# JosephCatrambone/aruco3

Hardware: AMD Instinct MI355X
Metric: frames/sec at 1920x1080 ARUCO dict (higher is better)
Workload: dtype u8

## Files before the change

aruco3_amd/_lib.py:

```python
import ctypes as C
from pathlib import Path

import numpy as np

import os

_HERE = Path(__file__).resolve().parent
LIB_PATH = Path(os.environ["A3_HIP_LIB"]).resolve() if os.environ.get("A3_HIP_LIB") else _HERE / "libaruco3_hip.so"

OK, ERR_INVALID, ERR_HIP, ERR_CAPACITY, ERR_INTERNAL, ERR_NO_DEVICE, ERR_LIMIT = 0, -1, -2, -3, -4, -5, -6
FMT_RGB8, FMT_RGBA8, FMT_L8, FMT_BGRA8 = 0, 1, 2, 3
MEM_HOST, MEM_DEVICE = 0, 1
PROFILE_OFF, PROFILE_STAGES, PROFILE_THRESHOLD_ONLY, PROFILE_THRESHOLD_SAMPLED = 0, 1, 2, 3
STAGE_THRESHOLD, STAGE_CONTOUR, STAGE_DECODE = 0, 1, 2
STEP_WHOLE, STEP_DECODE_DEFERRED, STEP_HELD_RELEASED_BY_LAST, STEP_HELD_RELEASED_EARLY, STEP_BURST_LAST, STEP_HELD = 0, 1, 2, 3, 4, 5
REFINE_NONE, REFINE_SUBPIX = 0, 1
BOARD_NONE, BOARD_OK = 0, 1
BOARD_MAX_MARKERS = 1024
DIST_NONE, DIST_RATIONAL = 0, 1
CHARUCO_MAX_CORNERS = 2048
CHARUCO_NO_ADJ = 0xFFFFFFFF
CALIB_FIX_PRINCIPAL_POINT, CALIB_ZERO_TANGENT_DIST, CALIB_FIX_K3, CALIB_RATIONAL_MODEL, CALIB_USE_INTRINSIC_GUESS = 1, 2, 4, 8, 16
CALIB_OK, CALIB_TOO_FEW, CALIB_NO_INIT, CALIB_NOT_FINITE = 1, 2, 3, 4
CALIB_VIEW_USED, CALIB_VIEW_TOO_FEW_POINTS, CALIB_VIEW_DEGENERATE = 1, 2, 3
# ... 6 lines not shown
STEP_NAMES = {0: "whole", 1: "decode_deferred", 2: "held_released_by_last", 3: "held_released_early", 4: "burst_last", 5: "held"}

SYMBOLS = [
    "a3_abi_version", "a3_default_config", "a3_create", "a3_destroy", "a3_last_error", "a3_set_stream", "a3_get_stream", "a3_set_pool_limits",
    "a3_get_tau", "a3_order_after", "a3_set_debug_taps", "a3_detect_batch", "a3_detect_batch_pose", "a3_detect_batch_submit", "a3_detect_batch_collect", "a3_detect_batch_pose_submit", "a3_detect_batch_pose_collect",
    "a3_host_alloc", "a3_host_free", "a3_host_register", "a3_host_unregister", "a3_get_stats", "a3_synth_render", "a3_download_grey", "a3_download_thresholded",
    "a3_candidate_count", "a3_download_candidates", "a3_download_homographies", "a3_estimate_pose", "a3_estimate_pose_normalized",
    "a3_find_nearest", "a3_calculate_tau", "a3_set_profiling", "a3_get_profile",
    "a3_contour_count", "a3_download_contours", "a3_detection_record_bytes", "a3_pack_detections",
    "a3_default_refine_config", "a3_set_corner_refinement", "a3_get_refined_corners", "a3_refine_corners",
    "a3_set_board", "a3_get_board_poses", "a3_estimate_board_pose",
    "a3_default_distortion", "a3_set_distortion", "a3_get_undistorted_corners", "a3_undistort_points",
    "a3_default_charuco_config", "a3_set_charuco", "a3_get_charuco_corners", "a3_get_charuco_poses", "a3_interpolate_charuco",
    "a3_calibrate_cameras", "a3_calibrate_rigs",
]
INTERNAL_SYMBOLS = ["a3_debug_set_overlap", "a3_debug_build_flags", "a3_debug_spin", "a3_debug_set_hold", "a3_debug_set_jump_rounds", "a3_debug_launch_threshold", "a3_debug_kernel_time", "a3_selftest_ieee", "a3_debug_clockwise", "a3_debug_rotate_bits", "a3_debug_discard_too_near", "a3_debug_inject_candidates"]


class A3Error(RuntimeError):
    def __init__(self, code, message):
        super().__init__(f"aruco3_hip error {code}: {message}")
        self.code = code


class Config(C.Structure):
    _fields_ = [
        ("threshold_window", C.c_uint32),
        ("contour_simplification_epsilon", C.c_double),
        ("min_side_length_factor", C.c_float),
        ("min_corner_separation_factor", C.c_float),
        ("homography_sample_size", C.c_uint32),
# ... 180 lines not shown
    L.a3_synth_render.restype = C.c_int
    L.a3_synth_render.argtypes = [C.c_int, vp, vp, C.c_uint32, vp, C.c_uint32, C.c_uint32, C.c_uint32, C.c_int, C.c_float, C.c_float, C.c_int,
                                  vp, C.c_size_t, C.c_size_t]
    if hasattr(L, "a3_debug_set_overlap"):
        L.a3_debug_set_overlap.restype = C.c_int
        L.a3_debug_set_overlap.argtypes = [C.c_int]
    if hasattr(L, "a3_debug_launch_threshold"):
        L.a3_debug_launch_threshold.restype = C.c_int
        L.a3_debug_launch_threshold.argtypes = [vp, vp, C.c_int, C.c_uint32, C.c_uint32, C.c_uint32]
    if hasattr(L, "a3_debug_set_hold"):
        L.a3_debug_set_hold.restype = C.c_int
        L.a3_debug_set_hold.argtypes = [C.c_int]
    if hasattr(L, "a3_debug_set_jump_rounds"):
        L.a3_debug_set_jump_rounds.restype = C.c_int
        L.a3_debug_set_jump_rounds.argtypes = [C.c_int]
    if hasattr(L, "a3_debug_spin"):
        L.a3_debug_spin.restype = C.c_int
        L.a3_debug_spin.argtypes = [vp, C.c_int, C.c_int, C.c_int]
    if hasattr(L, "a3_debug_build_flags"):
        L.a3_debug_build_flags.restype = C.c_int
        L.a3_debug_build_flags.argtypes = []
    L.a3_debug_kernel_time.restype = C.c_int
    L.a3_debug_kernel_time.argtypes = [vp, C.c_int, C.c_int, C.c_int, C.POINTER(C.c_float)]
    L.a3_get_stats.restype = C.c_int
    L.a3_get_stats.argtypes = [vp, C.POINTER(Stats)]
    L.a3_download_grey.restype = C.c_int
    L.a3_download_grey.argtypes = [vp, C.c_uint32, u8p]
    L.a3_download_thresholded.restype = C.c_int
    L.a3_download_thresholded.argtypes = [vp, C.c_uint32, u8p]
    L.a3_candidate_count.restype = C.c_int
# ... 546 lines not shown
```

aruco3_amd/csrc/a3_api.hip:

```cpp
#include <algorithm>
#include <atomic>
#include <cmath>
#include <chrono>
#include <cstddef>
#include <cstdio>
#include <cstring>
#include <mutex>
#include <string>
#include <vector>

#include "a3_common.h"
#include "a3_internal.h"

namespace a3 {
hipError_t launch_grey_threshold(hipStream_t, const uint8_t*, int, size_t, size_t, int, int, uint32_t, uint32_t, uint8_t*, uint64_t*, uint16_t*);
bool threshold_writes_grey_plane(uint32_t radius, const uint8_t* pixels, size_t row_stride, size_t frame_stride, int W);
hipError_t launch_dart_count(hipStream_t, const uint64_t*, int, int, uint32_t, uint32_t, unsigned long long*, uint32_t*, uint64_t, uint32_t*, uint32_t*, void*, size_t);
size_t tile_darts_bytes(uint32_t W, uint32_t H, uint32_t n_frames);
size_t tile_off_offset(uint32_t W, uint32_t H, uint32_t n_frames);
size_t tile_mask_offset_bytes(uint32_t W, uint32_t H, uint32_t n_frames);
hipError_t launch_dart_build(hipStream_t, const uint64_t*, int, int, uint32_t, uint32_t, const uint32_t*, const uint32_t*, uint32_t*, const uint32_t*,
                             uint64_t*, uint32_t*, uint32_t, const uint32_t*, int, const unsigned long long*);
hipError_t launch_zero(hipStream_t, void*, size_t);
size_t entry_state_bytes();
bool finalize_inline(bool frame_entries, bool trust_natural);
size_t fin_state_bytes();
size_t entry_slots(uint32_t);
size_t leader_list_bytes(uint32_t);
hipError_t launch_rank_cycles(hipStream_t, uint32_t, int, const uint64_t*, const uint32_t*,
                              uint32_t*, unsigned int*, void*, void*, void*, uint32_t*, unsigned int*, int, DeviceCounters*, const uint32_t*, int,
                              const uint32_t*, uint32_t*, uint32_t, int, uint32_t, unsigned int*, int);
hipError_t launch_resolve(hipStream_t, const void*, uint32_t, int, const uint64_t*, const uint32_t*, const unsigned int*, uint64_t*, uint64_t*,
                          DeviceCounters*, int, const uint32_t*);
hipError_t launch_select_scatter(hipStream_t, const void*, uint32_t, const uint32_t*, const unsigned int*, const uint32_t*, const uint64_t*,
                                 const uint32_t*, uint32_t, uint32_t,
                                 uint32_t, double, double, ContourRec*, uint32_t*, uint32_t, uint64_t, DeviceCounters*,
                                 const uint64_t*, uint32_t*, const uint32_t*, int, uint32_t*, int, const void*);
// ... 123 lines not shown
    int back_rc = 0;
    bool allow_defer = false;
    int batch_mode = 0;
    std::atomic<uint32_t> stepping{0};
    uint32_t released_others = 0;
    uint32_t reruns = 0;
    a3_config cfg{};
    uint8_t num_bits = 0, tau = 0;
    uint32_t n_codes = 0, mark_size = 0;
    std::string err;

    uint64_t max_darts = kMaxDartsDefault, max_points = kMaxPointsDefault;
    uint32_t max_contours = kMaxContoursDefault;
    uint32_t max_cand = kMaxCandDefault;
    int jump_rounds_hint = 10, resolve_iters_hint = 4;
    uint32_t dbg_nd = 0, dbg_frames = 0, dbg_chunks = 0;
    PixelSrc dbg_src{};
    std::vector<CandRec> inject;
    bool inject_armed = false;
    uint32_t inject_count = 0;
    Batch batch;
    bool pending_trivial = false;
    int resolve_full_ttl = 0;
    int entry_global_ttl = 0;
    bool plan_valid = false, force_host_plan = false;
    uint32_t plan_n = 0, plan_W = 0, plan_H = 0;
    uint64_t plan_darts = 0;
    bool debug_taps = false;
    uint32_t patch_cap = 0;
    bool grey_valid = false;
// ... 131 lines not shown
    A3_HIP(ctx->t_next.ensure(darts * 8));
    A3_HIP(ctx->leader_list.ensure(leader_list_bytes((uint32_t)darts)));
    A3_HIP(ctx->leader_keep.ensure(leader_list_bytes((uint32_t)darts)));
    const size_t eslots = entry_slots((uint32_t)darts);
    A3_HIP(ctx->entry_list.ensure(eslots * 4));
    A3_HIP(ctx->es_a.ensure(eslots * entry_state_bytes()));
    A3_HIP(ctx->es_b.ensure(eslots * entry_state_bytes()));
    return A3_OK;
}

struct DeviceStreams { hipStream_t decode = nullptr, copy = nullptr; };
std::mutex g_streams_mu;
DeviceStreams g_dev_streams[64];
bool g_hold_rests = true;
std::atomic<int> g_jump_rounds_cap{0};
enum { kStreamCopy = 0, kStreamDecode = 1 };

hipError_t create_stream(hipStream_t* st) { return hipStreamCreateWithPriority(st, hipStreamNonBlocking, 0); }

hipError_t device_stream(int device, int kind, hipStream_t* out) {
    std::lock_guard<std::mutex> lk(g_streams_mu);
    DeviceStreams& ds = g_dev_streams[device & 63];
    hipStream_t& st = kind == kStreamDecode ? ds.decode : ds.copy;
    if (!st) {
        const hipError_t e = create_stream(&st);
        if (e != hipSuccess) { st = nullptr; return e; }
    }
    *out = st;
    return hipSuccess;
}
// ... 347 lines not shown
    };
    std::vector<Chunk> chunks;
    std::vector<uint64_t> fd;
    if (device_plan) {
        if (int rc = ensure_chain_buffers(ctx, st, b, cap_d)) return rc;
        chunks.push_back(Chunk{0, n, cap_d, (uint32_t)std::min<uint64_t>(cap_d, 0xFFFFFFFFu)});
        A3_HIP(layout_zero_block(1, n, false));
        ctx->frame_darts_ptr = ctx->frame_darts_dev.as<unsigned long long>();
    } else {
        A3_HIP(ctx->tile_darts.ensure(tile_darts_bytes(W, H, n)));
        ctx->frame_darts_ptr = ctx->frame_darts.as<unsigned long long>();
        A3_HIP(hipMemsetAsync(ctx->frame_darts.p, 0, (size_t)n * 8, st));
    }
    A3_HIP(launch_dart_count(st, ctx->bin.as<uint64_t>(), (int)W, (int)H, 0, n, ctx->frame_darts_ptr, ctx->tile_darts.as<uint32_t>(), cap_d,
                             device_plan ? ctx->frame_base.as<uint32_t>() : nullptr, device_plan ? ctx->scratch_u32 + 8 : nullptr,
                             device_plan ? zero_p : nullptr, device_plan ? zero_bytes : 0));
    const uint32_t* n_live = device_plan ? ctx->scratch_u32 + 8 : nullptr;
    uint32_t max_chunk_frames = n;
    if (!device_plan) {
        if (int rc = ensure_pinned(ctx, std::max<size_t>((size_t)n * 8, 1 << 16))) return rc;
        A3_HIP(hipMemcpyAsync(ctx->pinned, ctx->frame_darts.p, (size_t)n * 8, hipMemcpyDeviceToHost, st));
        A3_HIP(wait_stream(st));
        fd.assign((uint64_t*)ctx->pinned, (uint64_t*)ctx->pinned + n);
        uint64_t biggest = 0;
        for (uint64_t v : fd) { biggest = std::max(biggest, v); ctx->stats.darts += v; }
        if (biggest > kHardMaxDarts) return fail(ctx, A3_ERR_LIMIT, "a frame needs more contour-graph nodes than 32-bit indices allow");
        if (biggest > ctx->max_darts) ctx->max_darts = biggest;
        Chunk c{0, 0, 0, 0};
        for (uint32_t f = 0; f < n; f++) {
            if (c.count && (c.darts + fd[f] > ctx->max_darts || c.count >= kMaxChunkFrames)) { chunks.push_back(c); c = Chunk{f, 0, 0, 0}; }
            c.count++; c.darts += fd[f]; c.max_frame_darts = (uint32_t)std::max<uint64_t>(c.max_frame_darts, fd[f]);
// ... 34 lines not shown
    const int resolve_iters = ctx->resolve_full_ttl > 0 ? ctx->resolve_iters_hint : 0;
    const int inline_resolve_W = ctx->resolve_full_ttl > 0 ? 0 : (int)W;
    const int keep_all = b.taps ? 1 : 0;
    int rounds_max = 0;
    for (size_t ci = 0; ci < chunks.size(); ci++) {
        const Chunk& c = chunks[ci];
        DeviceCounters* ctr = ctx->counters + ci;
        const uint32_t* fb = ctx->frame_base.as<uint32_t>() + ci * (max_chunk_frames + 1);
        const uint32_t nd = (uint32_t)c.darts;
        if (nd == 0) continue;
        if (ci > 0) {
            A3_HIP(hipMemsetAsync(d_leader_count, 0, 4 * 32, st));
            A3_HIP(hipMemsetAsync(ctx->frame_cursor, 0, (size_t)c.count * 4, st));
        }
        const uint32_t* tile_off = ctx->tile_darts.as<uint32_t>() + tile_off_offset(W, H, n);
        A3_HIP(launch_dart_build(st, d_bin, (int)W, (int)H, c.first, c.count, fb, tile_off, ctx->pix_base.as<uint32_t>(),
                                 ctx->tile_darts.as<uint32_t>(), ctx->d_xy.as<uint64_t>(), ctx->d_succ.as<uint32_t>(), nd, n_live, 0,
                                 reinterpret_cast<const unsigned long long*>(ctx->tile_darts.as<uint8_t>() + tile_mask_offset_bytes(W, H, n))));
        int rounds = 1;
        while ((1ull << rounds) < (uint64_t)c.max_frame_darts && rounds < 31) rounds++;
        rounds += 1;
        rounds = std::min(rounds, ctx->jump_rounds_hint);
        if (const int cap = g_jump_rounds_cap.load(std::memory_order_relaxed); cap > 0 && ctx->jump_rounds_hint < 32) rounds = std::min(rounds, cap);
        rounds_max = std::max(rounds_max, rounds);
        uint32_t* const frame_entries = ctx->entry_global_ttl > 0 ? nullptr : ctx->frame_cursor;
        const bool dense_graph = (uint64_t)nd * 10u >= (uint64_t)c.count * npx;
        unsigned int* const dead_ctr = (keep_all || !dense_graph) ? nullptr : d_dead_count;
        A3_HIP(launch_rank_cycles(st, nd, (int)W, ctx->d_xy.as<uint64_t>(), ctx->d_succ.as<uint32_t>(),
                                  ctx->entry_list.as<uint32_t>(), d_entry_count, ctx->es_a.p, ctx->es_b.p,
                                  ctx->fin.p, ctx->leader_list.as<uint32_t>(), d_leader_count, rounds, ctr, n_live, 0, fb,
                                  frame_entries, c.count, 1, min_edge_length, dead_ctr, inline_resolve_W > 0 ? 1 : 0));
        if (rel_mode == 2) { if (int rc = release_waiting()) return rc; }
        ctx->dbg_nd = nd; ctx->dbg_frames = c.count; ctx->dbg_chunks = (uint32_t)chunks.size();
// ... 63 lines not shown
    const float* h_undist = reinterpret_cast<const float*>(hp + head_bytes + (size_t)guess * (sizeof(a3_marker) + pose_bytes + refine_bytes) + board_bytes);
    const float* h_undist_res = h_undist + (size_t)guess * 8;
    {
        std::lock_guard<std::mutex> lk(g_defer_mu);
        if (int rc = flush_deferred_locked(ctx, nullptr)) return rc;
        if (const int rc = ctx->back_rc) { ctx->back_rc = 0; return rc; }
    }
    A3_HIP(wait_event(ctx->ev[4], st));
    const unsigned int* hs = reinterpret_cast<const unsigned int*>(hp);
    const DeviceCounters* hc = reinterpret_cast<const DeviceCounters*>(hp + 256);
    if (b.device_plan) {
        if (hs[9]) { ctx->force_host_plan = true; return 1; }
        ctx->stats.darts = hs[8];
        ctx->dbg_nd = hs[8];
        ctx->plan_darts = hs[8];
    } else {
        ctx->plan_valid = n_chunks == 1;
        ctx->plan_n = n; ctx->plan_W = b.W; ctx->plan_H = b.H;
        ctx->plan_darts = n_chunks == 1 ? b.chunk0_darts : 0;
    }
    unsigned int flags = hs[4];
    for (int sh = 0; sh < 16; sh++) ctx->stats.contours_traced += hs[48 + sh];
    uint64_t need_points = 0; uint32_t need_contours = 0;
    bool jump_short = false, resolve_needed = false, entry_overflow = false;
    for (size_t ci = 0; ci < n_chunks; ci++) {
        flags |= hc[ci].err_flags;
        resolve_needed |= hc[ci].resolve_needed != 0;
        entry_overflow |= hc[ci].entry_overflow != 0;
        need_points = std::max<uint64_t>(need_points, hc[ci].points);
        need_contours = std::max(need_contours, hc[ci].contours);
        ctx->stats.contours_traced += hc[ci].traced;
// ... 582 lines not shown
    struct EventPair {
        hipEvent_t e0 = nullptr, e1 = nullptr;
        ~EventPair() { if (e0) (void)hipEventDestroy(e0); if (e1) (void)hipEventDestroy(e1); }
    } evp;
    A3_HIP(hipEventCreate(&evp.e0)); A3_HIP(hipEventCreate(&evp.e1));
    const hipEvent_t e0 = evp.e0, e1 = evp.e1;
    double total = 0.0;
    unsigned int* d_entry_count = ctx->scratch_u32 + 32;
    unsigned int* d_leader_count = ctx->scratch_u32 + 16;
    for (int r = 0; r < reps; r++) {
        A3_HIP(hipMemsetAsync(d_leader_count, 0, 4 * 32, st));
        A3_HIP(hipEventRecord(e0, st));
        if (kernel == 0) {
            A3_HIP(hipMemsetAsync(ctx->frame_darts.p, 0, (size_t)ctx->frames * 8, st));
            A3_HIP(launch_dart_count(st, ctx->bin.as<uint64_t>(), (int)ctx->W, (int)ctx->H, 0, ctx->frames, ctx->frame_darts.as<unsigned long long>(),
                                     ctx->tile_darts.as<uint32_t>(), 0, nullptr, nullptr, nullptr, 0));
        } else if (kernel == 1) {
            A3_HIP(launch_dart_build(st, ctx->bin.as<uint64_t>(), (int)ctx->W, (int)ctx->H, 0, ctx->dbg_frames, ctx->frame_base.as<uint32_t>(),
                                     ctx->tile_darts.as<uint32_t>() + tile_off_offset(ctx->W, ctx->H, ctx->frames), ctx->pix_base.as<uint32_t>(),
                                     ctx->tile_darts.as<uint32_t>(), ctx->d_xy.as<uint64_t>(),
                                     ctx->d_succ.as<uint32_t>(), ctx->dbg_nd, nullptr, dbg ? dbg : 5,
                                     reinterpret_cast<const unsigned long long*>(ctx->tile_darts.as<uint8_t>() + tile_mask_offset_bytes(ctx->W, ctx->H, ctx->frames))));
        } else if (kernel == 2) {
            A3_HIP(launch_rank_cycles(st, ctx->dbg_nd, (int)ctx->W, ctx->d_xy.as<uint64_t>(), ctx->d_succ.as<uint32_t>(),
                                      ctx->entry_list.as<uint32_t>(),
                                      d_entry_count, ctx->es_a.p, ctx->es_b.p, ctx->fin.p,
                                      ctx->leader_list.as<uint32_t>(), d_leader_count, 0, ctx->counters, nullptr, dbg ? dbg : 11, ctx->frame_base.as<uint32_t>(), nullptr, ctx->dbg_frames, 0,
                                      0u, nullptr, 0));
        } else if (kernel == 3 || kernel == 4) {
            if (kernel == 4) {
                const size_t sweep = std::min<size_t>(ctx->pix_base.cap & ~(size_t)15, (size_t)512 << 20);
                if (sweep) A3_HIP(launch_zero(st, ctx->pix_base.p, sweep));
                A3_HIP(hipEventRecord(e0, st));
            }
            A3_HIP(launch_decode(st, ctx->dbg_src, (int)ctx->W, (int)ctx->H, 0, ctx->fin_xy.as<uint16_t>(), ctx->work.as<uint32_t>(), ctx->scratch_u32,
                                 ctx->max_cand, ctx->cfg.homography_sample_size, ctx->mark_size, ctx->cfg.homography_sample_size, ctx->dict.as<uint64_t>(),
                                 ctx->n_codes, ctx->tau, ctx->cfg.filter_high_bit_errors, ctx->proj.p, ctx->wtab.as<float>(), ctx->outs.p, nullptr, 0u, nullptr, 4096,
// ... 46 lines not shown
    return A3_OK;
}

int a3_debug_set_hold(int on) {
    std::lock_guard<std::mutex> lk(g_defer_mu);
    if (!g_held.empty()) return A3_ERR_INVALID;
    g_hold_rests = on != 0;
    return A3_OK;
}

int a3_debug_set_jump_rounds(int rounds) {
    if (rounds < 0 || rounds > 32) return A3_ERR_INVALID;
    g_jump_rounds_cap.store(rounds, std::memory_order_relaxed);
    return A3_OK;
}

int a3_synth_render(int device, void* hip_stream, const a3_synth_frame* frames, uint32_t n_frames, const a3_synth_marker* markers,
                    uint32_t n_markers, uint32_t width, uint32_t height, int paper, float black, float white, int supersample,
                    void* out_rgb_device, size_t row_stride, size_t frame_stride) {
    if (!frames || !out_rgb_device || (n_markers && !markers) || supersample < 1 || supersample > 8) return A3_ERR_INVALID;
    if (n_frames == 0 || width == 0 || height == 0) return A3_OK;
    if (row_stride == 0) row_stride = (size_t)width * 3;
    if (frame_stride == 0) frame_stride = row_stride * height;
    if (row_stride < (size_t)width * 3 || frame_stride < row_stride * (height - 1) + (size_t)width * 3 || height > 65535 || n_frames > 65535)
        return A3_ERR_INVALID;
    for (uint32_t f = 0; f < n_frames; f++)
        if ((uint64_t)frames[f].first_marker + frames[f].n_markers > n_markers) return A3_ERR_INVALID;
    for (uint32_t m = 0; m < n_markers; m++)
        if (markers[m].n == 0 || markers[m].n > 11) return A3_ERR_INVALID;
    if (hipSetDevice(device) != hipSuccess) return A3_ERR_NO_DEVICE;
// ... 859 lines not shown
```

aruco3_amd/csrc/a3_internal.h:

```cpp
#ifndef ARUCO3_HIP_INTERNAL_H
#define ARUCO3_HIP_INTERNAL_H

#include "../../include/aruco3_hip.h"

#ifdef __cplusplus
extern "C" {
#endif

int  a3_debug_kernel_time(a3_ctx *ctx, int kernel, int dbg, int reps, float *avg_ms);

int  a3_debug_set_overlap(int mode);

int  a3_debug_spin(void *hip_stream, int workgroups, int threads, int usec);

int  a3_debug_set_hold(int on);

int  a3_debug_set_jump_rounds(int rounds);

int  a3_debug_launch_threshold(a3_ctx *ctx, const void *pixels_device, int fmt, uint32_t width, uint32_t height, uint32_t n_frames);

int  a3_debug_build_flags(void);

int  a3_selftest_ieee(a3_ctx *ctx, const double *a, const double *b, size_t n, double *sqrt_a, double *a_div_b,
                      float *sqrtf_a, float *a_divf_b);

int  a3_debug_clockwise(a3_ctx *ctx, const int32_t *quads_xy, size_t n, int32_t *out_xy);
int  a3_debug_rotate_bits(a3_ctx *ctx, const uint8_t *bits, uint32_t n, uint32_t times, uint8_t *out);
int  a3_debug_inject_candidates(a3_ctx *ctx, const uint32_t *quads_xy, size_t n);
int  a3_debug_discard_too_near(a3_ctx *ctx, const uint32_t *quads_xy, size_t n, float min_distance, uint32_t *out_xy, size_t *n_out);

#ifdef __cplusplus
}
#endif
// ... 2 lines not shown
```

aruco3_amd/csrc/k_contours.hip:

```cpp
#include <algorithm>

#include "a3_common.h"


namespace a3 {

constexpr int kFinB = 8;
constexpr int kScatB = 1;

struct Nb8 { uint64_t c; uint64_t n[8]; };

__device__ __forceinline__ uint64_t ldw(const uint64_t* __restrict__ img, int wpr, int H, int j, int y) {
    return (y >= 0 && y < H && j >= 0 && j < wpr) ? img[(size_t)y * wpr + j] : 0ull;
}

__device__ __forceinline__ void pdart_words(const Nb8& nb, uint64_t p[8]) {
#pragma unroll
    for (int k = 0; k < 8; k++) {
        uint64_t m = nb.c & nb.n[k] & ~nb.n[(k + 7) & 7];
        if ((k & 1) == 0) m &= ~nb.n[(k + 6) & 7];
        p[k] = m;
    }
}

// ... 56 lines not shown
    r.n[1] = (a << 1) | (al >> 63);
    r.n[2] = a;
    r.n[3] = (a >> 1) | (ar << 63);
    r.n[4] = (c >> 1) | (cr << 63);
    r.n[5] = (b >> 1) | (br << 63);
    r.n[6] = b;
    r.n[7] = (b << 1) | (bl >> 63);
    return r;
}

constexpr int kCountLanes = 60;
constexpr int kCountHalves = 4;
template <int G>
__global__ __launch_bounds__(64) void k_dart_count(const uint64_t* __restrict__ bits, int W, int H, uint32_t first_frame,
                                                   unsigned long long* __restrict__ frame_darts, uint32_t* __restrict__ tile_darts,
                                                   uint32_t* __restrict__ tile_darts_h1, unsigned long long* __restrict__ tile_mask) {
    static_assert(kCountLanes % kTileWords == 0, "a wave counts whole tiles");
    static_assert((kTileRows / kCountHalves) * kTileWords == 64, "one 64-bit mask per tile and part");
    constexpr int kGroups = 64 / G, kOwners = G == 64 ? kCountLanes : 30, kTilesPerGroup = (kOwners + kTileWords - 1) / kTileWords;
    __shared__ uint32_t s_tile[kGroups][kTilesPerGroup];
    __shared__ unsigned long long s_mask[kGroups][kTilesPerGroup];
    constexpr uint32_t kQ = 128;
    __shared__ uint64_t q_c[kQ], q_up[kQ], q_dn[kQ];
    __shared__ uint32_t q_meta[kQ];
    const int wpr = (int)words_per_row((uint32_t)W);
    const uint32_t f = blockIdx.y;
    const uint32_t tiles_x = dart_tiles_x((uint32_t)W), tiles_y = ((uint32_t)H + kTileRows - 1) / kTileRows;
    const int chunks_x = G == 64 ? (wpr + kCountLanes - 1) / kCountLanes : 1;
    const int lane = threadIdx.x, gl = lane & (G - 1), grp = lane / G;
    const int cx = blockIdx.x % chunks_x, ty = (blockIdx.x / chunks_x) * kGroups + grp;
    const int j = cx * kOwners + gl - 1;
    const bool owner = gl >= 1 && gl <= kOwners && j < wpr && ty < (int)tiles_y;
    const uint64_t* img = bits + (size_t)(first_frame + f) * wpr * H;
    if (lane < kGroups * kTilesPerGroup) { (&s_tile[0][0])[lane] = 0; (&s_mask[0][0])[lane] = 0ull; }
    constexpr int kRows = kTileRows / kCountHalves;
    const int y0 = ty * kTileRows + (int)blockIdx.z * kRows;
    const int jc = min(max(j, 0), wpr - 1);
    auto word = [&](int y) -> uint64_t {
        const uint64_t v = img[(size_t)min(max(y, 0), H - 1) * wpr + jc];
        return v & (0ull - (uint64_t)(y >= 0 && y < H && j >= 0 && j < wpr));
    };
    auto edge_bits = [](uint64_t c, uint32_t* lr) {
        const uint32_t l = (uint32_t)__builtin_amdgcn_update_dpp(0, (int)(uint32_t)(c >> 32), 0x138 , 0xF, 0xF, true) >> 31;
        const uint32_t r = (uint32_t)__builtin_amdgcn_update_dpp(0, (int)(uint32_t)c, 0x130 , 0xF, 0xF, true) & 1u;
        *lr = l | (r << 1);
    };
    struct Row3 { uint64_t c; uint32_t lr; };
    constexpr int kAhead = 16;
    static_assert(kRows % kAhead == 0, "whole batches of rows");
    Row3 up, cur;
    uint64_t nxt[kAhead], ahead[kAhead];
    up.c = word(y0 - 1);
    cur.c = word(y0);
#pragma unroll
    for (int u = 0; u < kAhead; u++) nxt[u] = word(y0 + u + 1);
    edge_bits(up.c, &up.lr);
    edge_bits(cur.c, &cur.lr);
    uint32_t qhead = 0, qtail = 0;
    const uint32_t lane_row0 = (uint32_t)lane << 8;
    auto work = [&](uint32_t slot) {
        const uint64_t c = q_c[slot], uc = q_up[slot], dc = q_dn[slot];
        const uint32_t m = q_meta[slot];
        Nb8 nb;
        nb.c = c;
        nb.n[0] = (c << 1) | (m & 1u);                  nb.n[4] = (c >> 1) | ((uint64_t)((m >> 1) & 1u) << 63);
        nb.n[1] = (uc << 1) | ((m >> 2) & 1u);          nb.n[3] = (uc >> 1) | ((uint64_t)((m >> 3) & 1u) << 63);
        nb.n[2] = uc;                                   nb.n[6] = dc;
        nb.n[7] = (dc << 1) | ((m >> 4) & 1u);          nb.n[5] = (dc >> 1) | ((uint64_t)((m >> 5) & 1u) << 63);
        uint64_t p[8];
        pdart_words(nb, p);
// ... 92 lines not shown
    if (threadIdx.x == 0) {
        const unsigned long long total = s_run;
        const bool fits = total <= cap;
        frame_base[n_frames] = fits ? (uint32_t)total : 0u;
        plan[0] = fits ? (uint32_t)total : 0u;
        plan[1] = fits ? 0u : 1u;
        plan[2] = s_max;
        plan[3] = (uint32_t)min(total, 0xFFFFFFFFull);
    }
}

__global__ __launch_bounds__(256) void k_tile_scan(uint32_t* __restrict__ tile_darts, const uint32_t* __restrict__ tile_darts_h1, uint32_t tiles, uint32_t first_frame,
                                                   uint32_t* __restrict__ tile_off, uint32_t n_frames,
                                                   unsigned long long* __restrict__ frame_darts, unsigned long long cap,
                                                   uint32_t* __restrict__ frame_base, uint32_t* __restrict__ plan,
                                                   uint4* __restrict__ zero_p, uint32_t zero_n16) {
    if (blockIdx.x == n_frames) {
        for (uint32_t i = threadIdx.x; i < zero_n16; i += 256) zero_p[i] = make_uint4(0u, 0u, 0u, 0u);
        __syncthreads();
        plan_frames(frame_darts, n_frames, cap, frame_base, plan);
        return;
    }
    __shared__ uint32_t s_wave[4];
    __shared__ uint32_t s_run;
    const size_t base = (size_t)(first_frame + blockIdx.x) * tiles;
    if (threadIdx.x == 0) s_run = 0;
    __syncthreads();
    for (uint32_t t0 = 0; t0 < tiles; t0 += 256) {
        const uint32_t t = t0 + threadIdx.x;
        uint32_t v = 0;
        if (t < tiles) {
            v = tile_darts[base + t];
#pragma unroll
            for (int z = 1; z < kCountHalves; z++) v += tile_darts_h1[(size_t)(z - 1) * n_frames * tiles + base + t];
        }
        if (t < tiles) tile_darts[base + t] = v;
        uint32_t total;
        const uint32_t excl = block_excl_scan_256(v, s_wave, &total);
        if (t < tiles) tile_off[base + t] = s_run + excl;
        __syncthreads();
        if (threadIdx.x == 0) s_run += total;
        __syncthreads();
    }
}

__device__ __forceinline__ uint32_t row3(uint64_t l, uint64_t c, uint64_t r, int i) {
    const uint64_t v = i == 0 ? ((c << 1) | (l >> 63)) : (c >> (i - 1));
    return ((uint32_t)v & 7u) | (i == 63 ? ((uint32_t)r & 1u) << 2 : 0u);
}
__device__ __forceinline__ uint32_t tile_F(const uint64_t (*s_t)[kTileWords + 2], int rl, int jl, int i) {
    const uint32_t* base = reinterpret_cast<const uint32_t*>(&s_t[0][0]);
    const int p1 = (jl + 1) * 64 + i - 1, d = p1 >> 5, sh = p1 & 31;
    constexpr int kRowDwords = 2 * (kTileWords + 2);
    uint32_t rows[3];
// ... 25 lines not shown
        if (!(F & 16u)) {
            const uint32_t rr = ((F >> 5) | (F << 3)) & 0xFFu;
            uint32_t first = 0;
            for (uint32_t b = 0; b < 8; b++) if (rr & (1u << b)) { first = b + 1; break; }
            kE = (5 + first - 1) & 7;
        }
        t.v[F] = (uint16_t)(P | (kW << 8) | (kE << 12));
    }
    return t;
}
__device__ __constant__ const PixLut kPixLut = make_pix_lut();

__device__ __forceinline__ int dir_dx(int k) { return (int)((0x1A90u >> (2 * k)) & 3u) - 1; }
__device__ __forceinline__ int dir_dy(int k) { return (int)((0xA901u >> (2 * k)) & 3u) - 1; }

__global__ __launch_bounds__(256) void k_dart_assign(const uint64_t* __restrict__ bits, int W, int H, uint32_t first_frame,
                                                     const uint32_t* __restrict__ frame_base, const uint32_t* __restrict__ tile_off,
                                                     uint32_t* __restrict__ pix_base, const uint32_t* __restrict__ tile_darts,
                                                     uint64_t* __restrict__ d_rec, uint32_t* __restrict__ d_succ,
                                                     const uint32_t* __restrict__ n_live, int dbg,
                                                     const unsigned long long* __restrict__ tile_mask, uint32_t tiles, uint32_t n_frames) {
    __shared__ uint32_t s_wave[4];
    __shared__ uint64_t s_t[kTileRows + 2][kTileWords + 2];
    __shared__ uint64_t s_nodes[256];
    __shared__ uint64_t s_c0[256], s_c1[256], s_c2[256];
    __shared__ uint32_t s_dbase[256];
    __shared__ uint32_t s_mark[512];
    __shared__ uint16_t s_nbk[256];
    __shared__ uint8_t s_wofrank[256], s_rank[256], s_fr[256];
    __shared__ uint32_t s_multi;
    __shared__ uint16_t s_lut[256];
    const int wpr = (int)words_per_row((uint32_t)W);
    const uint32_t n_wg = tiles * n_frames, chunk = (n_wg + 7u) >> 3, g = (blockIdx.x & 7u) * chunk + (blockIdx.x >> 3);
    if (g >= n_wg) return;
    const uint32_t f = g / tiles, tile = g - f * tiles;
    if (tile_darts[(size_t)(first_frame + f) * tiles + tile] == 0u) return;
    if (n_live && *n_live == 0u) return;
    const uint32_t dart0 = frame_base[f] + tile_off[(size_t)(first_frame + f) * tiles + tile];
    if (dbg == 1) return;
    __shared__ uint32_t s_cnt[256];
    const unsigned long long* tm = tile_mask + ((size_t)(first_frame + f) * tiles + tile) * kCountHalves;
    static_assert(kCountHalves == 4 && kTileWords == 4 && kTileRows == 64, "four 64-bit word masks per tile, four word columns of 64 rows");
    unsigned long long cm[4];
#pragma unroll
    for (int c = 0; c < 4; c++)
        cm[c] = ((tm[0] >> (16 * c)) & 0xFFFFull) | (((tm[1] >> (16 * c)) & 0xFFFFull) << 16) | (((tm[2] >> (16 * c)) & 0xFFFFull) << 32) | (((tm[3] >> (16 * c)) & 0xFFFFull) << 48);
    const unsigned long long m0 = cm[0], m1 = cm[1], m2 = cm[2], m3 = cm[3];
    tile_stage(bits + (size_t)(first_frame + f) * wpr * H, W, H, tile, s_t);
    s_cnt[threadIdx.x] = 0;
    s_mark[threadIdx.x] = 0; s_mark[256 + threadIdx.x] = 0;
    s_lut[threadIdx.x] = kPixLut.v[threadIdx.x];
    if (threadIdx.x == 0) s_multi = 0;
// ... 80 lines not shown
                    const uint64_t below2 = (1ull << i2) - 1ull;
                    const uint32_t off2 = single ? (uint32_t)__popcll(s_nodes[w2] & below2)
                                                 : (uint32_t)__popcll(s_c0[w2] & below2) + 2u * (uint32_t)__popcll(s_c1[w2] & below2) +
                                                   4u * (uint32_t)__popcll(s_c2[w2] & below2);
                    succ = dart0 + s_dbase[w2] + off2 + (uint32_t)__popc(P2 & ((1u << kin) - 1u));
                }
            } else {
                succ = kNone;
            }
            if (dbg != 4 || succ == 0x12345678u) d_succ[cur] = succ;
            cur++;
        }
    }
}

__device__ __forceinline__ uint32_t pixel_F(const uint64_t* __restrict__ img, int wpr, int H, int x, int y) {
    const int j = x >> 6, i = x & 63;
    uint32_t rows[3];
#pragma unroll
    for (int dy = -1; dy <= 1; dy++) {
        const uint64_t c = ldw(img, wpr, H, j, y + dy);
        const uint64_t l = i == 0 ? ldw(img, wpr, H, j - 1, y + dy) : 0ull;
        const uint64_t r = i == 63 ? ldw(img, wpr, H, j + 1, y + dy) : 0ull;
        rows[dy + 1] = row3(l, c, r, i);
    }
    const uint32_t top = rows[0], mid = rows[1], bot = rows[2];
    return (mid & 1u) | ((top & 7u) << 1) | ((mid & 4u) << 2) | ((bot & 4u) << 3) | ((bot & 2u) << 5) | ((bot & 1u) << 7);
}

__device__ __forceinline__ uint32_t cross_tile_succ(uint32_t d, uint64_t rec, int W, int H, int wpr, uint32_t first_frame,
// ... 1018 lines not shown
    if (b < 1) b = 1;
    if (b > (uint64_t)cap) b = cap;
    return (int)b;
}

__global__ __launch_bounds__(256) void k_zero(uint4* __restrict__ p, uint32_t n16) {
    for (uint32_t i = blockIdx.x * blockDim.x + threadIdx.x; i < n16; i += gridDim.x * blockDim.x) p[i] = make_uint4(0u, 0u, 0u, 0u);
}
hipError_t launch_zero(hipStream_t st, void* p, size_t bytes ) {
    const uint32_t n16 = (uint32_t)(bytes / 16);
    hipLaunchKernelGGL(k_zero, dim3(blocks_for(n16, 256, 256)), dim3(256), 0, st, reinterpret_cast<uint4*>(p), n16);
    return hipGetLastError();
}

size_t tile_mask_offset_bytes(uint32_t W, uint32_t H, uint32_t n_frames);
size_t tile_darts_bytes(uint32_t W, uint32_t H, uint32_t n_frames) { return tile_mask_offset_bytes(W, H, n_frames) + (size_t)dart_tiles(W, H) * n_frames * kCountHalves * 8; }
size_t tile_off_offset(uint32_t W, uint32_t H, uint32_t n_frames) { return (size_t)dart_tiles(W, H) * n_frames; }
size_t tile_mask_offset_bytes(uint32_t W, uint32_t H, uint32_t n_frames) { return ((size_t)dart_tiles(W, H) * n_frames * 4 * (1 + kCountHalves) + 7) & ~(size_t)7; }

hipError_t launch_dart_count(hipStream_t st, const uint64_t* bits, int W, int H, uint32_t first_frame, uint32_t n_frames,
                             unsigned long long* frame_darts, uint32_t* tile_darts, uint64_t plan_cap, uint32_t* frame_base, uint32_t* plan,
                             void* zero_p, size_t zero_bytes ) {
    const uint32_t tiles_x = dart_tiles_x((uint32_t)W), tiles_y = ((uint32_t)H + kTileRows - 1) / kTileRows;
    const uint32_t wpr = words_per_row((uint32_t)W);
    uint32_t* h1 = tile_darts + (size_t)tiles_x * tiles_y * n_frames * 2;
    unsigned long long* tmask = reinterpret_cast<unsigned long long*>(reinterpret_cast<uint8_t*>(tile_darts) + tile_mask_offset_bytes((uint32_t)W, (uint32_t)H, n_frames));
    if (wpr <= 30)
        hipLaunchKernelGGL(k_dart_count<32>, dim3((tiles_y + 1) / 2, n_frames, kCountHalves), dim3(64), 0, st, bits, W, H, first_frame, frame_darts, tile_darts, h1, tmask);
    else
        hipLaunchKernelGGL(k_dart_count<64>, dim3(((wpr + kCountLanes - 1) / kCountLanes) * tiles_y, n_frames, kCountHalves), dim3(64), 0, st, bits, W, H, first_frame,
                           frame_darts, tile_darts, h1, tmask);
    hipLaunchKernelGGL(k_tile_scan, dim3(n_frames + (plan ? 1u : 0u)), dim3(256), 0, st, tile_darts, h1, tiles_x * tiles_y, first_frame,
                       tile_darts + (size_t)tiles_x * tiles_y * n_frames, n_frames, frame_darts, (unsigned long long)plan_cap, frame_base, plan,
                       reinterpret_cast<uint4*>(zero_p), (uint32_t)(zero_bytes / 16));
    return hipGetLastError();
}

hipError_t launch_dart_build(hipStream_t st, const uint64_t* bits, int W, int H, uint32_t first_frame, uint32_t n_frames,
                             const uint32_t* frame_base, const uint32_t* tile_off, uint32_t* pix_base, const uint32_t* tile_darts, uint64_t* d_rec,
                             uint32_t* d_succ, uint32_t n_darts, const uint32_t* n_live, int dbg, const unsigned long long* tile_mask) {
    const uint32_t tiles = dart_tiles((uint32_t)W, (uint32_t)H);
    hipLaunchKernelGGL(k_dart_assign, dim3((tiles * n_frames + 7u) / 8u * 8u), dim3(256), 0, st, bits, W, H, first_frame, frame_base, tile_off,
                       pix_base, tile_darts, d_rec, d_succ, n_live, dbg, tile_mask, tiles, n_frames);
    if (dbg && dbg != 5) return hipGetLastError();
    hipLaunchKernelGGL(k_dart_link, dim3(blocks_for(n_darts, 256, 4096)), dim3(256), 0, st, W, H, first_frame, pix_base, bits, d_rec, d_succ, n_darts, n_live);
    return hipGetLastError();
}

size_t entry_state_bytes() { return sizeof(EntryState); }
bool finalize_inline(bool frame_entries, bool trust_natural) { return frame_entries && trust_natural; }
size_t fin_state_bytes() { return sizeof(FinState); }
size_t entry_slots(uint32_t n_darts) { return (size_t)entry_shard_cap(n_darts) * kEntryShards; }
size_t leader_list_bytes(uint32_t n_darts) { return (size_t)leader_shard_cap(n_darts) * kLeaderShards * 4; }

hipError_t launch_rank_cycles(hipStream_t st, uint32_t n_darts, int W, const uint64_t* d_rec, const uint32_t* d_succ,
                              uint32_t* entry_list,
                              unsigned int* entry_count, void* es_a, void* es_b, void* fin8 , uint32_t* leader_list,
                              unsigned int* leader_count, int max_rounds, DeviceCounters* ctr, const uint32_t* n_live, int dbg,
// ... 103 lines not shown
```

Baseline: 386,800.

## Compact non-empty dart tiles into a list and size assign grid from it

The tile scan now builds a compacted list of tiles with nonzero dart counts, using an atomic counter. A new listed assign kernel walks only that list with a grid-stride loop, and its grid is sized from the previous call's listed count plus slack. The old path launched one workgroup per tile and returned early on empty tiles. Separately, the dart-count kernel gets an interior fast path that skips clamped, bounds-checked row loads. The costs are extra scan and atomic work, a larger buffer, and a grid hint that depends on the previous frame.

```diff
diff --git a/aruco3_amd/_lib.py b/aruco3_amd/_lib.py
--- a/aruco3_amd/_lib.py
+++ b/aruco3_amd/_lib.py
@@ -44,7 +44,7 @@
     "a3_default_charuco_config", "a3_set_charuco", "a3_get_charuco_corners", "a3_get_charuco_poses", "a3_interpolate_charuco",
     "a3_calibrate_cameras", "a3_calibrate_rigs",
 ]
-INTERNAL_SYMBOLS = ["a3_debug_set_overlap", "a3_debug_build_flags", "a3_debug_spin", "a3_debug_set_hold", "a3_debug_set_jump_rounds", "a3_debug_launch_threshold", "a3_debug_kernel_time", "a3_selftest_ieee", "a3_debug_clockwise", "a3_debug_rotate_bits", "a3_debug_discard_too_near", "a3_debug_inject_candidates"]
+INTERNAL_SYMBOLS = ["a3_debug_set_overlap", "a3_debug_build_flags", "a3_debug_spin", "a3_debug_set_hold", "a3_debug_set_jump_rounds", "a3_debug_set_assign_grid", "a3_debug_assign_listed", "a3_debug_launch_threshold", "a3_debug_kernel_time", "a3_selftest_ieee", "a3_debug_clockwise", "a3_debug_rotate_bits", "a3_debug_discard_too_near", "a3_debug_inject_candidates"]
 
 
 class A3Error(RuntimeError):
@@ -255,6 +255,12 @@
     if hasattr(L, "a3_debug_set_jump_rounds"):
         L.a3_debug_set_jump_rounds.restype = C.c_int
         L.a3_debug_set_jump_rounds.argtypes = [C.c_int]
+    if hasattr(L, "a3_debug_set_assign_grid"):
+        L.a3_debug_set_assign_grid.restype = C.c_int
+        L.a3_debug_set_assign_grid.argtypes = [C.c_int]
+    if hasattr(L, "a3_debug_assign_listed"):
+        L.a3_debug_assign_listed.restype = C.c_longlong
+        L.a3_debug_assign_listed.argtypes = [vp]
     if hasattr(L, "a3_debug_spin"):
         L.a3_debug_spin.restype = C.c_int
         L.a3_debug_spin.argtypes = [vp, C.c_int, C.c_int, C.c_int]
diff --git a/aruco3_amd/csrc/a3_api.hip b/aruco3_amd/csrc/a3_api.hip
--- a/aruco3_amd/csrc/a3_api.hip
+++ b/aruco3_amd/csrc/a3_api.hip
@@ -15,12 +15,13 @@
 namespace a3 {
 hipError_t launch_grey_threshold(hipStream_t, const uint8_t*, int, size_t, size_t, int, int, uint32_t, uint32_t, uint8_t*, uint64_t*, uint16_t*);
 bool threshold_writes_grey_plane(uint32_t radius, const uint8_t* pixels, size_t row_stride, size_t frame_stride, int W);
-hipError_t launch_dart_count(hipStream_t, const uint64_t*, int, int, uint32_t, uint32_t, unsigned long long*, uint32_t*, uint64_t, uint32_t*, uint32_t*, void*, size_t);
+hipError_t launch_dart_count(hipStream_t, const uint64_t*, int, int, uint32_t, uint32_t, unsigned long long*, uint32_t*, uint64_t, uint32_t*, uint32_t*, void*, size_t, bool);
 size_t tile_darts_bytes(uint32_t W, uint32_t H, uint32_t n_frames);
 size_t tile_off_offset(uint32_t W, uint32_t H, uint32_t n_frames);
 size_t tile_mask_offset_bytes(uint32_t W, uint32_t H, uint32_t n_frames);
+size_t tile_list_offset_bytes(uint32_t W, uint32_t H, uint32_t n_frames);
 hipError_t launch_dart_build(hipStream_t, const uint64_t*, int, int, uint32_t, uint32_t, const uint32_t*, const uint32_t*, uint32_t*, const uint32_t*,
-                             uint64_t*, uint32_t*, uint32_t, const uint32_t*, int, const unsigned long long*);
+                             uint64_t*, uint32_t*, uint32_t, const uint32_t*, int, const unsigned long long*, const uint32_t*, uint32_t, uint32_t*);
 hipError_t launch_zero(hipStream_t, void*, size_t);
 size_t entry_state_bytes();
 bool finalize_inline(bool frame_entries, bool trust_natural);
@@ -174,6 +175,7 @@
     uint32_t max_contours = kMaxContoursDefault;
     uint32_t max_cand = kMaxCandDefault;
     int jump_rounds_hint = 10, resolve_iters_hint = 4;
+    int64_t assign_listed_hint = -1;
     uint32_t dbg_nd = 0, dbg_frames = 0, dbg_chunks = 0;
     PixelSrc dbg_src{};
     std::vector<CandRec> inject;
@@ -335,6 +337,7 @@
 DeviceStreams g_dev_streams[64];
 bool g_hold_rests = true;
 std::atomic<int> g_jump_rounds_cap{0};
+std::atomic<int> g_assign_grid_cap{0};
 enum { kStreamCopy = 0, kStreamDecode = 1 };
 
 hipError_t create_stream(hipStream_t* st) { return hipStreamCreateWithPriority(st, hipStreamNonBlocking, 0); }
@@ -712,7 +715,7 @@
     }
     A3_HIP(launch_dart_count(st, ctx->bin.as<uint64_t>(), (int)W, (int)H, 0, n, ctx->frame_darts_ptr, ctx->tile_darts.as<uint32_t>(), cap_d,
                              device_plan ? ctx->frame_base.as<uint32_t>() : nullptr, device_plan ? ctx->scratch_u32 + 8 : nullptr,
-                             device_plan ? zero_p : nullptr, device_plan ? zero_bytes : 0));
+                             device_plan ? zero_p : nullptr, device_plan ? zero_bytes : 0, device_plan));
     const uint32_t* n_live = device_plan ? ctx->scratch_u32 + 8 : nullptr;
     uint32_t max_chunk_frames = n;
     if (!device_plan) {
@@ -777,9 +780,14 @@
             A3_HIP(hipMemsetAsync(ctx->frame_cursor, 0, (size_t)c.count * 4, st));
         }
         const uint32_t* tile_off = ctx->tile_darts.as<uint32_t>() + tile_off_offset(W, H, n);
+        uint32_t assign_grid = 0;
+        if (device_plan && ctx->assign_listed_hint >= 0) assign_grid = (uint32_t)std::min<int64_t>(ctx->assign_listed_hint + ctx->assign_listed_hint / 16 + 64, 0x7FFFFFFF);
+        if (const int cap = g_assign_grid_cap.load(std::memory_order_relaxed); device_plan && cap > 0) assign_grid = assign_grid ? std::min(assign_grid, (uint32_t)cap) : (uint32_t)cap;
         A3_HIP(launch_dart_build(st, d_bin, (int)W, (int)H, c.first, c.count, fb, tile_off, ctx->pix_base.as<uint32_t>(),
                                  ctx->tile_darts.as<uint32_t>(), ctx->d_xy.as<uint64_t>(), ctx->d_succ.as<uint32_t>(), nd, n_live, 0,
-                                 reinterpret_cast<const unsigned long long*>(ctx->tile_darts.as<uint8_t>() + tile_mask_offset_bytes(W, H, n))));
+                                 reinterpret_cast<const unsigned long long*>(ctx->tile_darts.as<uint8_t>() + tile_mask_offset_bytes(W, H, n)),
+                                 device_plan ? reinterpret_cast<const uint32_t*>(ctx->tile_darts.as<uint8_t>() + tile_list_offset_bytes(W, H, n)) : nullptr,
+                                 assign_grid, device_plan ? ctx->scratch_u32 + 12 : nullptr));
         int rounds = 1;
         while ((1ull << rounds) < (uint64_t)c.max_frame_darts && rounds < 31) rounds++;
         rounds += 1;
@@ -873,7 +881,9 @@
         ctx->stats.darts = hs[8];
         ctx->dbg_nd = hs[8];
         ctx->plan_darts = hs[8];
+        ctx->assign_listed_hint = hs[12];
     } else {
+        ctx->assign_listed_hint = -1;
         ctx->plan_valid = n_chunks == 1;
         ctx->plan_n = n; ctx->plan_W = b.W; ctx->plan_H = b.H;
         ctx->plan_darts = n_chunks == 1 ? b.chunk0_darts : 0;
@@ -1486,13 +1496,14 @@
         if (kernel == 0) {
             A3_HIP(hipMemsetAsync(ctx->frame_darts.p, 0, (size_t)ctx->frames * 8, st));
             A3_HIP(launch_dart_count(st, ctx->bin.as<uint64_t>(), (int)ctx->W, (int)ctx->H, 0, ctx->frames, ctx->frame_darts.as<unsigned long long>(),
-                                     ctx->tile_darts.as<uint32_t>(), 0, nullptr, nullptr, nullptr, 0));
+                                     ctx->tile_darts.as<uint32_t>(), 0, nullptr, nullptr, nullptr, 0, false));
         } else if (kernel == 1) {
             A3_HIP(launch_dart_build(st, ctx->bin.as<uint64_t>(), (int)ctx->W, (int)ctx->H, 0, ctx->dbg_frames, ctx->frame_base.as<uint32_t>(),
                                      ctx->tile_darts.as<uint32_t>() + tile_off_offset(ctx->W, ctx->H, ctx->frames), ctx->pix_base.as<uint32_t>(),
                                      ctx->tile_darts.as<uint32_t>(), ctx->d_xy.as<uint64_t>(),
                                      ctx->d_succ.as<uint32_t>(), ctx->dbg_nd, nullptr, dbg ? dbg : 5,
-                                     reinterpret_cast<const unsigned long long*>(ctx->tile_darts.as<uint8_t>() + tile_mask_offset_bytes(ctx->W, ctx->H, ctx->frames))));
+                                     reinterpret_cast<const unsigned long long*>(ctx->tile_darts.as<uint8_t>() + tile_mask_offset_bytes(ctx->W, ctx->H, ctx->frames)),
+                                     nullptr, 0, nullptr));
         } else if (kernel == 2) {
             A3_HIP(launch_rank_cycles(st, ctx->dbg_nd, (int)ctx->W, ctx->d_xy.as<uint64_t>(), ctx->d_succ.as<uint32_t>(),
                                       ctx->entry_list.as<uint32_t>(),
@@ -1569,6 +1580,14 @@
     g_jump_rounds_cap.store(rounds, std::memory_order_relaxed);
     return A3_OK;
 }
+
+int a3_debug_set_assign_grid(int workgroups) {
+    if (workgroups < 0) return A3_ERR_INVALID;
+    g_assign_grid_cap.store(workgroups, std::memory_order_relaxed);
+    return A3_OK;
+}
+
+long long a3_debug_assign_listed(const a3_ctx* ctx) { return ctx ? (long long)ctx->assign_listed_hint : -1; }
 
 int a3_synth_render(int device, void* hip_stream, const a3_synth_frame* frames, uint32_t n_frames, const a3_synth_marker* markers,
                     uint32_t n_markers, uint32_t width, uint32_t height, int paper, float black, float white, int supersample,
diff --git a/aruco3_amd/csrc/a3_internal.h b/aruco3_amd/csrc/a3_internal.h
--- a/aruco3_amd/csrc/a3_internal.h
+++ b/aruco3_amd/csrc/a3_internal.h
@@ -17,6 +17,9 @@
 
 int  a3_debug_set_jump_rounds(int rounds);
 
+int  a3_debug_set_assign_grid(int workgroups);
+long long a3_debug_assign_listed(const a3_ctx *ctx);
+
 int  a3_debug_launch_threshold(a3_ctx *ctx, const void *pixels_device, int fmt, uint32_t width, uint32_t height, uint32_t n_frames);
 
 int  a3_debug_build_flags(void);
diff --git a/aruco3_amd/csrc/k_contours.hip b/aruco3_amd/csrc/k_contours.hip
--- a/aruco3_amd/csrc/k_contours.hip
+++ b/aruco3_amd/csrc/k_contours.hip
@@ -94,7 +94,9 @@
 template <int G>
 __global__ __launch_bounds__(64) void k_dart_count(const uint64_t* __restrict__ bits, int W, int H, uint32_t first_frame,
                                                    unsigned long long* __restrict__ frame_darts, uint32_t* __restrict__ tile_darts,
-                                                   uint32_t* __restrict__ tile_darts_h1, unsigned long long* __restrict__ tile_mask) {
+                                                   uint32_t* __restrict__ tile_darts_h1, unsigned long long* __restrict__ tile_mask,
+                                                   uint32_t* __restrict__ list_count) {
+    if (list_count && (blockIdx.x | blockIdx.y | blockIdx.z) == 0u && threadIdx.x == 0) *list_count = 0u;
     static_assert(kCountLanes % kTileWords == 0, "a wave counts whole tiles");
     static_assert((kTileRows / kCountHalves) * kTileWords == 64, "one 64-bit mask per tile and part");
     constexpr int kGroups = 64 / G, kOwners = G == 64 ? kCountLanes : 30, kTilesPerGroup = (kOwners + kTileWords - 1) / kTileWords;
@@ -120,6 +122,13 @@
         const uint64_t v = img[(size_t)min(max(y, 0), H - 1) * wpr + jc];
         return v & (0ull - (uint64_t)(y >= 0 && y < H && j >= 0 && j < wpr));
     };
+    const bool inner = __all(y0 >= 1 && y0 + kRows < H) != 0 && (uint64_t)wpr * (uint64_t)H * 8u < (1ull << 32);
+    const uint64_t col_mask = 0ull - (uint64_t)(j >= 0 && j < wpr);
+    const uint32_t lane_off = ((uint32_t)(y0 - 1) * (uint32_t)wpr + (uint32_t)jc) * 8u;
+    auto word_inner = [&](int d) -> uint64_t {
+        const char* row = reinterpret_cast<const char*>(img) + (size_t)d * (size_t)wpr * 8u;
+        return *reinterpret_cast<const uint64_t*>(row + lane_off) & col_mask;
+    };
     auto edge_bits = [](uint64_t c, uint32_t* lr) {
         const uint32_t l = (uint32_t)__builtin_amdgcn_update_dpp(0, (int)(uint32_t)(c >> 32), 0x138 , 0xF, 0xF, true) >> 31;
         const uint32_t r = (uint32_t)__builtin_amdgcn_update_dpp(0, (int)(uint32_t)c, 0x130 , 0xF, 0xF, true) & 1u;
@@ -130,10 +139,17 @@
     static_assert(kRows % kAhead == 0, "whole batches of rows");
     Row3 up, cur;
     uint64_t nxt[kAhead], ahead[kAhead];
-    up.c = word(y0 - 1);
-    cur.c = word(y0);
-#pragma unroll
-    for (int u = 0; u < kAhead; u++) nxt[u] = word(y0 + u + 1);
+    if (inner) {
+        up.c = word_inner(0);
+        cur.c = word_inner(1);
+#pragma unroll
+        for (int u = 0; u < kAhead; u++) nxt[u] = word_inner(u + 2);
+    } else {
+        up.c = word(y0 - 1);
+        cur.c = word(y0);
+#pragma unroll
+        for (int u = 0; u < kAhead; u++) nxt[u] = word(y0 + u + 1);
+    }
     edge_bits(up.c, &up.lr);
     edge_bits(cur.c, &cur.lr);
     uint32_t qhead = 0, qtail = 0;
@@ -256,15 +272,16 @@
                                                    uint32_t* __restrict__ tile_off, uint32_t n_frames,
                                                    unsigned long long* __restrict__ frame_darts, unsigned long long cap,
                                                    uint32_t* __restrict__ frame_base, uint32_t* __restrict__ plan,
-                                                   uint4* __restrict__ zero_p, uint32_t zero_n16) {
+                                                   uint4* __restrict__ zero_p, uint32_t zero_n16,
+                                                   uint32_t* __restrict__ tile_list, uint32_t* __restrict__ list_count) {
     if (blockIdx.x == n_frames) {
         for (uint32_t i = threadIdx.x; i < zero_n16; i += 256) zero_p[i] = make_uint4(0u, 0u, 0u, 0u);
         __syncthreads();
         plan_frames(frame_darts, n_frames, cap, frame_base, plan);
         return;
     }
-    __shared__ uint32_t s_wave[4];
-    __shared__ uint32_t s_run;
+    __shared__ uint32_t s_wave[4], s_wave_l[4];
+    __shared__ uint32_t s_run, s_lbase;
     const size_t base = (size_t)(first_frame + blockIdx.x) * tiles;
     if (threadIdx.x == 0) s_run = 0;
     __syncthreads();
@@ -280,6 +297,13 @@
         uint32_t total;
         const uint32_t excl = block_excl_scan_256(v, s_wave, &total);
         if (t < tiles) tile_off[base + t] = s_run + excl;
+        if (tile_list) {
+            uint32_t n_own;
+            const uint32_t k = block_excl_scan_256(v != 0u ? 1u : 0u, s_wave_l, &n_own);
+            if (threadIdx.x == 0 && n_own) s_lbase = atomicAdd(list_count, n_own);
+            __syncthreads();
+            if (v) tile_list[s_lbase + k] = blockIdx.x * tiles + t;
+        }
         __syncthreads();
         if (threadIdx.x == 0) s_run += total;
         __syncthreads();
@@ -335,12 +359,10 @@
 __device__ __forceinline__ int dir_dx(int k) { return (int)((0x1A90u >> (2 * k)) & 3u) - 1; }
 __device__ __forceinline__ int dir_dy(int k) { return (int)((0xA901u >> (2 * k)) & 3u) - 1; }
 
-__global__ __launch_bounds__(256) void k_dart_assign(const uint64_t* __restrict__ bits, int W, int H, uint32_t first_frame,
-                                                     const uint32_t* __restrict__ frame_base, const uint32_t* __restrict__ tile_off,
-                                                     uint32_t* __restrict__ pix_base, const uint32_t* __restrict__ tile_darts,
-                                                     uint64_t* __restrict__ d_rec, uint32_t* __restrict__ d_succ,
-                                                     const uint32_t* __restrict__ n_live, int dbg,
-                                                     const unsigned long long* __restrict__ tile_mask, uint32_t tiles, uint32_t n_frames) {
+__device__ __forceinline__ void dart_assign_tile(const uint64_t* __restrict__ bits, int W, int H, uint32_t first_frame,
+                                                 const uint32_t* __restrict__ frame_base, const uint32_t* __restrict__ tile_off,
+                                                 uint32_t* __restrict__ pix_base, uint64_t* __restrict__ d_rec, uint32_t* __restrict__ d_succ,
+                                                 int dbg, const unsigned long long* __restrict__ tile_mask, uint32_t tiles, uint32_t f, uint32_t tile) {
     __shared__ uint32_t s_wave[4];
     __shared__ uint64_t s_t[kTileRows + 2][kTileWords + 2];
     __shared__ uint64_t s_nodes[256];
@@ -352,11 +374,6 @@
     __shared__ uint32_t s_multi;
     __shared__ uint16_t s_lut[256];
     const int wpr = (int)words_per_row((uint32_t)W);
-    const uint32_t n_wg = tiles * n_frames, chunk = (n_wg + 7u) >> 3, g = (blockIdx.x & 7u) * chunk + (blockIdx.x >> 3);
-    if (g >= n_wg) return;
-    const uint32_t f = g / tiles, tile = g - f * tiles;
-    if (tile_darts[(size_t)(first_frame + f) * tiles + tile] == 0u) return;
-    if (n_live && *n_live == 0u) return;
     const uint32_t dart0 = frame_base[f] + tile_off[(size_t)(first_frame + f) * tiles + tile];
     if (dbg == 1) return;
     __shared__ uint32_t s_cnt[256];
@@ -467,6 +484,39 @@
     }
 }
 
+__global__ __launch_bounds__(256) void k_dart_assign(const uint64_t* __restrict__ bits, int W, int H, uint32_t first_frame,
+                                                     const uint32_t* __restrict__ frame_base, const uint32_t* __restrict__ tile_off,
+                                                     uint32_t* __restrict__ pix_base, const uint32_t* __restrict__ tile_darts,
+                                                     uint64_t* __restrict__ d_rec, uint32_t* __restrict__ d_succ,
+                                                     const uint32_t* __restrict__ n_live, int dbg,
+                                                     const unsigned long long* __restrict__ tile_mask, uint32_t tiles, uint32_t n_frames) {
+    const uint32_t n_wg = tiles * n_frames, chunk = (n_wg + 7u) >> 3, g = (blockIdx.x & 7u) * chunk + (blockIdx.x >> 3);
+    if (g >= n_wg) return;
+    const uint32_t f = g / tiles, tile = g - f * tiles;
+    if (tile_darts[(size_t)(first_frame + f) * tiles + tile] == 0u) return;
+    if (n_live && *n_live == 0u) return;
+    dart_assign_tile(bits, W, H, first_frame, frame_base, tile_off, pix_base, d_rec, d_succ, dbg, tile_mask, tiles, f, tile);
+}
+
+__global__ __launch_bounds__(256) void k_dart_assign_listed(const uint64_t* __restrict__ bits, int W, int H, uint32_t first_frame,
+                                                            const uint32_t* __restrict__ frame_base, const uint32_t* __restrict__ tile_off,
+                                                            uint32_t* __restrict__ pix_base, uint64_t* __restrict__ d_rec, uint32_t* __restrict__ d_succ,
+                                                            const uint32_t* __restrict__ n_live, const unsigned long long* __restrict__ tile_mask,
+                                                            uint32_t tiles, const uint32_t* __restrict__ tile_list,
+                                                            const uint32_t* __restrict__ list_count, uint32_t* __restrict__ listed_out) {
+    const uint32_t n_items = *list_count, live = *n_live;
+    const uint32_t chunk = (n_items + 7u) >> 3, per_xcd = gridDim.x >> 3;
+    if (blockIdx.x == 0 && threadIdx.x == 0) *listed_out = n_items;
+    if (live == 0u) return;
+    for (uint32_t s = blockIdx.x >> 3; s < chunk; s += per_xcd) {
+        const uint32_t g = (blockIdx.x & 7u) * chunk + s;
+        if (g >= n_items) break;
+        const uint32_t ft = tile_list[g], f = ft / tiles;
+        dart_assign_tile(bits, W, H, first_frame, frame_base, tile_off, pix_base, d_rec, d_succ, 0, tile_mask, tiles, f, ft - f * tiles);
+        __syncthreads();
+    }
+}
+
 __device__ __forceinline__ uint32_t pixel_F(const uint64_t* __restrict__ img, int wpr, int H, int x, int y) {
     const int j = x >> 6, i = x & 63;
     uint32_t rows[3];
@@ -1515,34 +1565,44 @@
 }
 
 size_t tile_mask_offset_bytes(uint32_t W, uint32_t H, uint32_t n_frames);
-size_t tile_darts_bytes(uint32_t W, uint32_t H, uint32_t n_frames) { return tile_mask_offset_bytes(W, H, n_frames) + (size_t)dart_tiles(W, H) * n_frames * kCountHalves * 8; }
+size_t tile_list_offset_bytes(uint32_t W, uint32_t H, uint32_t n_frames) { return tile_mask_offset_bytes(W, H, n_frames) + (size_t)dart_tiles(W, H) * n_frames * kCountHalves * 8; }
+size_t tile_darts_bytes(uint32_t W, uint32_t H, uint32_t n_frames) { return tile_list_offset_bytes(W, H, n_frames) + 16 + (size_t)dart_tiles(W, H) * n_frames * 4; }
 size_t tile_off_offset(uint32_t W, uint32_t H, uint32_t n_frames) { return (size_t)dart_tiles(W, H) * n_frames; }
 size_t tile_mask_offset_bytes(uint32_t W, uint32_t H, uint32_t n_frames) { return ((size_t)dart_tiles(W, H) * n_frames * 4 * (1 + kCountHalves) + 7) & ~(size_t)7; }
 
 hipError_t launch_dart_count(hipStream_t st, const uint64_t* bits, int W, int H, uint32_t first_frame, uint32_t n_frames,
                              unsigned long long* frame_darts, uint32_t* tile_darts, uint64_t plan_cap, uint32_t* frame_base, uint32_t* plan,
-                             void* zero_p, size_t zero_bytes ) {
+                             void* zero_p, size_t zero_bytes , bool list) {
     const uint32_t tiles_x = dart_tiles_x((uint32_t)W), tiles_y = ((uint32_t)H + kTileRows - 1) / kTileRows;
     const uint32_t wpr = words_per_row((uint32_t)W);
     uint32_t* h1 = tile_darts + (size_t)tiles_x * tiles_y * n_frames * 2;
     unsigned long long* tmask = reinterpret_cast<unsigned long long*>(reinterpret_cast<uint8_t*>(tile_darts) + tile_mask_offset_bytes((uint32_t)W, (uint32_t)H, n_frames));
+    uint32_t* lcount = list ? reinterpret_cast<uint32_t*>(reinterpret_cast<uint8_t*>(tile_darts) + tile_list_offset_bytes((uint32_t)W, (uint32_t)H, n_frames)) : nullptr;
+    uint32_t* tlist = list ? lcount + 4 : nullptr;
     if (wpr <= 30)
-        hipLaunchKernelGGL(k_dart_count<32>, dim3((tiles_y + 1) / 2, n_frames, kCountHalves), dim3(64), 0, st, bits, W, H, first_frame, frame_darts, tile_darts, h1, tmask);
+        hipLaunchKernelGGL(k_dart_count<32>, dim3((tiles_y + 1) / 2, n_frames, kCountHalves), dim3(64), 0, st, bits, W, H, first_frame, frame_darts, tile_darts, h1, tmask, lcount);
     else
         hipLaunchKernelGGL(k_dart_count<64>, dim3(((wpr + kCountLanes - 1) / kCountLanes) * tiles_y, n_frames, kCountHalves), dim3(64), 0, st, bits, W, H, first_frame,
-                           frame_darts, tile_darts, h1, tmask);
+                           frame_darts, tile_darts, h1, tmask, lcount);
     hipLaunchKernelGGL(k_tile_scan, dim3(n_frames + (plan ? 1u : 0u)), dim3(256), 0, st, tile_darts, h1, tiles_x * tiles_y, first_frame,
                        tile_darts + (size_t)tiles_x * tiles_y * n_frames, n_frames, frame_darts, (unsigned long long)plan_cap, frame_base, plan,
-                       reinterpret_cast<uint4*>(zero_p), (uint32_t)(zero_bytes / 16));
+                       reinterpret_cast<uint4*>(zero_p), (uint32_t)(zero_bytes / 16), tlist, lcount);
     return hipGetLastError();
 }
 
 hipError_t launch_dart_build(hipStream_t st, const uint64_t* bits, int W, int H, uint32_t first_frame, uint32_t n_frames,
                              const uint32_t* frame_base, const uint32_t* tile_off, uint32_t* pix_base, const uint32_t* tile_darts, uint64_t* d_rec,
-                             uint32_t* d_succ, uint32_t n_darts, const uint32_t* n_live, int dbg, const unsigned long long* tile_mask) {
+                             uint32_t* d_succ, uint32_t n_darts, const uint32_t* n_live, int dbg, const unsigned long long* tile_mask,
+                             const uint32_t* listed , uint32_t grid_hint, uint32_t* listed_out) {
     const uint32_t tiles = dart_tiles((uint32_t)W, (uint32_t)H);
-    hipLaunchKernelGGL(k_dart_assign, dim3((tiles * n_frames + 7u) / 8u * 8u), dim3(256), 0, st, bits, W, H, first_frame, frame_base, tile_off,
-                       pix_base, tile_darts, d_rec, d_succ, n_live, dbg, tile_mask, tiles, n_frames);
+    uint32_t grid = (tiles * n_frames + 7u) / 8u * 8u;
+    if (listed) {
+        if (grid_hint) grid = std::min(grid, (grid_hint + 7u) / 8u * 8u);
+        hipLaunchKernelGGL(k_dart_assign_listed, dim3(grid), dim3(256), 0, st, bits, W, H, first_frame, frame_base, tile_off, pix_base, d_rec, d_succ,
+                           n_live, tile_mask, tiles, listed + 4, listed, listed_out);
+    } else
+        hipLaunchKernelGGL(k_dart_assign, dim3(grid), dim3(256), 0, st, bits, W, H, first_frame, frame_base, tile_off,
+                           pix_base, tile_darts, d_rec, d_succ, n_live, dbg, tile_mask, tiles, n_frames);
     if (dbg && dbg != 5) return hipGetLastError();
     hipLaunchKernelGGL(k_dart_link, dim3(blocks_for(n_darts, 256, 4096)), dim3(256), 0, st, W, H, first_frame, pix_base, bits, d_rec, d_succ, n_darts, n_live);
     return hipGetLastError();
```

Result: no change. 390,500, median of 6 (+1.0%).
